# l13039968960/stm32H7-YOLO

Measured on AMD Instinct MI355X. Metric: images/sec int8 YOLO-face 56x56, higher is better.
Workload: dtype int8; 1 GPU; BASELINE configs[1]: batch=4096 int8 YOLO-face 56x56x3 frames per GPU, fused LDS-resident forward + GPU box decode; frames_per_gpu=4096, global_batch=4096, frame_bytes_in=9408, frame_bytes_out=882, input_batches_rotated=8, input_bytes_resident=308281344, kernel=yoloface56_fused<F=2,NW=8>, requant_rounding=ref, parallelism=single GPU, gather_every=1, collectives_issued=0, launch_streams=2

## Files before the change

### stm32h7-yolo_amd/csrc/yf_fused56.hip.h

```cpp


template <class B, int C, int F, int NT>
__device__ __forceinline__ void dump_buf(const char* frames, int8_t* dump, long stride, long off, long first_frame,
                                         long n_frames, int tid, int ch0 = 0, int split = 1 << 30, int gap = 0) {
  if (!dump) return;
  for (int i = tid; i < F * B::P * C; i += NT) {
    const int ch = i % C; const int t = i / C;
    const int p = t % B::P; const int f = t / B::P;
    if (first_frame + f >= n_frames) continue;
    const int phys = ch0 + ch + (ch >= split ? gap : 0);
    dump[(first_frame + f) * stride + off + (long)p * C + ch] = (int8_t)frames[f * B::FS + B::at_p(p) + phys];
  }
}

template <class B, int C, int FT, int NT, class IdOf>
__device__ __forceinline__ void dump_sets(const char* frames, int8_t* dump, long stride, long off, const IdOf& id_of, int tid, int ch0 = 0, int split = 1 << 30, int gap = 0) {
  for (int i = tid; i < FT * B::P * C; i += NT) {
    const int ch = i % C; const int t = i / C;
    const int p = t % B::P; const int f = t / B::P;
    const long id = id_of(f);
    if (id < 0) continue;
    const int phys = ch0 + ch + (ch >= split ? gap : 0);
    dump[id * stride + off + (long)p * C + ch] = (int8_t)frames[f * B::FS + B::at_p(p) + phys];
  }
}

struct DumpOffsets {
  enum { T1 = 0, T2 = T1 + 6272, T3 = T2 + 6272, T4 = T3 + 3136, Q21 = T4 + 14112, T6 = Q21 + 3528, T7 = T6 + 3528,
         T8 = T7 + 1176, T9 = T8 + 7056, T11 = T9 + 7056, T14 = T11 + 1176, T15 = T14 + 7056, Q45 = T15 + 4704,
         T17 = Q45 + 1176, T18 = T17 + 1176, T19 = T18 + 392, T20 = T19 + 1960, T22 = T20 + 1960, T23 = T22 + 392,
         T24 = T23 + 1960, T26 = T24 + 1960, T30 = T26 + 392, T31 = T30 + 2352, T32 = T31 + 1960, T33 = T32 + 1960,
         P8 = T33 + 1568, C17 = P8 + 3528, P25 = C17 + 1176, C34 = P25 + 1176, C40 = C34 + 392, L43 = C40 + 392,
         TOTAL = L43 + 1176 };
};
// ... 44 lines not shown
#endif
template <bool DUMP> constexpr bool tail_batch() { return !DUMP || YF_PDUMP; }

template <int F, int NW, bool DUMP, bool CAM = false>
#if !defined(YF_LAB) || !defined(YF_TPJ13)
#undef YF_TPJ13
#define YF_TPJ13 3
#endif
#if !defined(YF_LAB) || !defined(YF_TPJ23)
#undef YF_TPJ23
#define YF_TPJ23 2
#endif
#if defined(YF_LAB) && defined(YF_WHATIF_WPE)
#define YF_WPE(NW) YF_WHATIF_WPE
#else
#define YF_WPE(NW) ((NW) == 12 ? 6 : (NW) >= 8 ? 4 : ((NW) == 6 ? 3 : 2))
#endif
__global__ void __launch_bounds__(NW * 64, YF_WPE(NW)) yoloface56_fused(const NetParams prm) {
  extern __shared__ __attribute__((aligned(16))) char smem[];
  constexpr int NT = NW * 64;
  constexpr bool BATCH = tail_batch<DUMP>();
  constexpr bool POOL_MERGE = YF_POOL_MERGE != 0 && (!DUMP || YF_PDUMP) && NW >= 8;
  constexpr bool XDUMP = DUMP && !YF_PDUMP;
  typedef Buf<B_T14::OFF, 14, 14, 32, 14, 0, 0> B_T6X;
  typedef typename std::conditional<POOL_MERGE, B_T6X, B_T6>::type B_T6M;
  constexpr int FT = BATCH ? 2 * F : F;
  typedef TailBufs<BATCH ? FRAME_STRIDE / 2 : FRAME_STRIDE> U;
  constexpr int OUT_ALL_BYTES = BATCH ? 0 : (F * OUT_FRAME_BYTES + 15) & ~15;
  static_assert(std::is_same<decltype(&yoloface56_fused<F, NW, DUMP, CAM>), void (*)(const NetParams)>::value, "YF_ARG: NetParams is the kernel's only argument (kernarg offset 0)");
  uint8_t* luts = reinterpret_cast<uint8_t*>(smem);
  constexpr int PRE = v2::pre_bytes<F, tail_batch<DUMP>()>();
  char* out_all = smem + PRE;
  char* frames = smem + PRE + OUT_ALL_BYTES;
  const int n_frames = (int)prm.n;
  const int tid0 = threadIdx.x;
  const uint8_t* __restrict__ tab = prm.tab;
  int vz = 0;
  asm volatile("" : "+v"(vz));
  const __attribute__((address_space(1))) uint8_t* lut_src = (const __attribute__((address_space(1))) uint8_t*)(tab + PLAN.lut_off);
  asm volatile("" : "+s"(lut_src));
  for (int i = tid0; i < v2::LUT_B / 16; i += NT)
    reinterpret_cast<v4u*>(luts)[i] = *(const __attribute__((address_space(1))) v4u*)(lut_src + (uint32_t)(16 * i));
  for (int i = tid0; i < v2::ZERO_B / 16; i += NT) reinterpret_cast<uint4*>(smem + v2::ZERO)[i] = uint4{0, 0, 0, 0};
  constexpr int DBG_LUT = PRE + OUT_ALL_BYTES + FRAME_BYTES + (F - 1) * FRAME_STRIDE;
  if constexpr (DUMP) { if (tid0 < YF_DBG_LUT_BYTES / 16) reinterpret_cast<v4u*>(smem + DBG_LUT)[tid0] = *(const __attribute__((address_space(1))) v4u*)(lut_src + (uint32_t)(YF_N_LUT * 256 + YF_ADDLUT_BYTES + 16 * tid0)); }
#if !(defined(YF_LAB) && defined(YF_WHATIF_NO_PROLOGUE_TABLES))
  {
// ... 385 lines not shown
```

### stm32h7-yolo_amd/csrc/yf_kernels.hip.h

```cpp
#include <hip/hip_runtime.h>
#include <stddef.h>
#include <stdint.h>
#include <type_traits>
#include "yf_tables.h"

#pragma clang diagnostic push
#pragma clang diagnostic ignored "-Wint-to-pointer-cast"
#if !defined(YF_LAB) || !defined(YF_LAUNDER)
#undef YF_LAUNDER
#define YF_LAUNDER 0
#endif
#define YF_ROW_SKEW 4
#define YF_T8_ROW_SKEW 32
namespace YF_NS {

#ifndef YF_NOINLINE_STAGES
#define YF_STAGE_FN __device__ __forceinline__
#else
#define YF_STAGE_FN __device__ __attribute__((noinline))
#endif

typedef int v4i __attribute__((ext_vector_type(4)));
typedef short v2s __attribute__((ext_vector_type(2)));

#if !defined(YF_H0) || YF_H0 == 56
constexpr int FRAME_BYTES = 34176;
#endif
constexpr int LUT_BYTES = YF_N_LUT * 256 + YF_ADDLUT_BYTES;


#if !defined(YF_H0) || YF_H0 == 56
#if defined(YF_LAB) && defined(YF_WHATIF_FS)
constexpr int FRAME_STRIDE = YF_WHATIF_FS;
#else
constexpr int FRAME_STRIDE = FRAME_BYTES;
#endif
constexpr int BUF_FS = FRAME_STRIDE;
#else
constexpr int BUF_FS = 0;
#endif
template <int OFF_, int W_, int H_, int S_, int RS_, int PT_, int PL_, int FS_ = BUF_FS, int SK_ = 0>
struct Buf {
  static constexpr int OFF = OFF_, W = W_, H = H_, S = S_, RS = RS_, PT = PT_, PL = PL_, FS = FS_, SK = SK_;
  static constexpr int P = W_ * H_, ROWB = RS_ * S_ + SK_;
  __device__ static __forceinline__ int at(int y, int x) { return OFF_ + (y + PT_) * ROWB + (x + PL_) * S_; }
  __device__ static __forceinline__ int at_p(int p) {
    if constexpr (RS_ == W_ && PT_ == 0 && PL_ == 0) return OFF_ + p * S_;
    else { const int y = p / W_; return at(y, p - y * W_); }
  }
};
template <int WIDTH>
constexpr bool lds_conflict_free(const int (&addr)[32]) {
  for (int i = 0; i < 32; ++i) {
    if (addr[i] % WIDTH != 0) return false;
    for (int j = 0; j < i; ++j)
      if (addr[i] != addr[j] && (addr[i] / WIDTH) % 32 == (addr[j] / WIDTH) % 32) return false;
  }
  return true;
}

#ifndef YF_H0
#define YF_H0 56
#endif
constexpr int G0 = YF_H0, G1 = G0 / 2, G2 = G0 / 4, G3 = G0 / 8;
static_assert(G0 % 8 == 0 && G3 >= 4, "input size must be a multiple of 8 and at least 32");

#if YF_H0 == 56
typedef Buf<    0, 56, 56,  4, 60, 1, 4> B_IN;
typedef Buf<13696, 28, 28,  8, 30, 1, 1, BUF_FS, YF_ROW_SKEW> B_T1;
typedef Buf<21024, 28, 28,  8, 28, 0, 0> B_T2;
typedef Buf<16832, 28, 28,  4, 28, 0, 0> B_T3;
typedef Buf<    0, 28, 28, 20, 29, 1, 1> B_T4;
typedef Buf<16832, 14, 28, 20, 14, 0, 0> B_HB;
typedef Buf<24672, 14, 14, 48, 14, 0, 0> B_T14;
typedef Buf<16832, 14, 14, 32, 14, 0, 0> B_T6;
typedef Buf<    0, 14, 14,  8, 14, 0, 0> B_T7;
typedef Buf< 1568, 14, 14, 36, 16, 1, 1, BUF_FS, YF_T8_ROW_SKEW> B_T8;
typedef Buf<11296, 14, 14, 48, 14, 0, 0> B_T9;
typedef Buf<20704, 14, 14,  8, 14, 0, 0> B_T11;
typedef Buf<    0, 14, 14, 24, 15, 1, 1> B_T15;
typedef Buf< 5408,  7,  7, 48,  7, 0, 0> B_T30;
typedef Buf< 7760,  7,  7, 32,  7, 0, 0> B_T17;
typedef Buf< 9328,  7,  7,  8,  7, 0, 0> B_T18;
typedef Buf< 9728,  7,  7, 40,  9, 1, 1, BUF_FS, YF_ROW_SKEW> B_T19;
typedef Buf<13008,  7,  7, 48,  7, 0, 0> B_T20;
typedef Buf<15360,  7,  7,  8,  7, 0, 0> B_T22;
typedef Buf<15752,  7,  7,  8,  7, 0, 0> B_T26;
typedef Buf<16144,  7,  7, 32,  7, 0, 0> B_T33;
template <int FS_>
struct TailBufs {
  typedef Buf<    0, 14, 14, 24, 15, 1, 1, FS_> T15;
  typedef Buf< 5408,  7,  7, 48,  7, 0, 0, FS_> T30;
  typedef Buf< 7760,  7,  7, 32,  7, 0, 0, FS_> T17;
  typedef Buf< 9328,  7,  7,  8,  7, 0, 0, FS_> T18;
  typedef Buf< 9728,  7,  7, 40,  9, 1, 1, FS_, YF_ROW_SKEW> T19;
  typedef Buf<13008,  7,  7, 48,  7, 0, 0, FS_> T20;
  typedef Buf<15360,  7,  7,  8,  7, 0, 0, FS_> T22;
  typedef Buf<15752,  7,  7,  8,  7, 0, 0, FS_> T26;
  typedef Buf< 7760,  7,  7, 32,  7, 0, 0, FS_> T33;
  typedef Buf<16160,  7,  7, 18,  7, 0, 0, FS_> HEAD;
  static constexpr int END = 16160 + 882, T15_BYTES = 5408;
  static_assert(T19::OFF + 9 * T19::ROWB <= T20::OFF && T20::OFF + 49 * 48 <= T22::OFF && T26::OFF + 49 * 8 <= HEAD::OFF, "tail buffers do not overlap");
#if !(defined(YF_LAB) && defined(YF_WHATIF_FS))
  static_assert(END <= FS_, "a set fits its stride");
#endif
};
#else
constexpr int arena_next(int off, int bytes) { return (off + bytes + 64 + 63) & ~63; }
#define YF_SEQ(NAME, PREV_END, W_, H_, S_, RS_, PT_, PL_, ROWS_)                      \
  constexpr int NAME##_OFF = PREV_END;                                                \
  typedef Buf<NAME##_OFF, W_, H_, S_, RS_, PT_, PL_> NAME;                            \
  constexpr int NAME##_END = arena_next(NAME##_OFF, (ROWS_) * (RS_) * (S_));
YF_SEQ(B_IN,  0,         G0, G0,  4, G0 + 4, 1, 4, G0 + 1)
YF_SEQ(B_T1,  B_IN_END,  G1, G1,  8, G1 + 2, 1, 1, G1 + 2)
// ... 246 lines not shown
template <int JOBS, int NW>
__device__ __forceinline__ void job_range(int wave, int& j0, int& j1) {
  constexpr int BASE = JOBS / NW, REM = JOBS % NW;
  j0 = wave * BASE + min(wave, REM);
  j1 = j0 + BASE + (wave < REM ? 1 : 0);
}

template <class B, bool RING, int F, int NT>
YF_STAGE_FN void fill_halo(char* frames, int zp, int tid) {
  const uint32_t v = (uint32_t)(zp & 255) * 0x01010101u;
  constexpr int DW = B::S / 4;
  constexpr int HR = B::H + B::PT + (RING ? 1 : 0), WR = B::RS;
  constexpr int NPIX = RING ? (2 * WR + 2 * (HR - 2)) : (WR + HR - 1);
  for (int i = tid; i < F * NPIX * DW; i += NT) {
    const int d = i % DW, t = i / DW, k = t % NPIX, f = t / NPIX;
    int r, c;
    if constexpr (RING) {
      if (k < WR) { r = 0; c = k; }
      else if (k < 2 * WR) { r = HR - 1; c = k - WR; }
      else { const int m = k - 2 * WR; r = 1 + (m >> 1); c = (m & 1) ? WR - 1 : 0; }
    } else {
      if (k < WR) { r = 0; c = k; } else { r = 1 + (k - WR); c = 0; }
    }
    *reinterpret_cast<uint32_t*>(frames + f * B::FS + B::OFF + r * B::ROWB + c * B::S + 4 * d) = v;
  }
}

__device__ __forceinline__ uint32_t funnel(uint32_t hi, uint32_t lo, int sh) { return __builtin_amdgcn_alignbit(hi, lo, sh); }
template <int F, int NT>
YF_STAGE_FN void stage_input(char* frames, const int8_t* __restrict__ in, int first_frame, int n_frames,
                                            int zp, int tid) {
  const uint32_t hv = (uint32_t)(zp & 255) * 0x01010101u;
  constexpr int RSW = B_IN::RS, HH = B_IN::H, WQ = B_IN::W / 4;
  constexpr int PER_FRAME = HH * WQ, TOTAL = F * PER_FRAME, ITERS = (TOTAL + NT - 1) / NT;
  for (int i = tid; i < F * (RSW + HH); i += NT) {
    const int f = i / (RSW + HH), k = i - f * (RSW + HH);
    const int idx = k < RSW ? k : (k - RSW + 1) * RSW + 3;
    *reinterpret_cast<uint32_t*>(frames + f * B_IN::FS + B_IN::OFF + idx * 4) = hv;
  }
  const int lastf = min(n_frames - 1 - first_frame, F - 1);
  const int8_t* base = in + (size_t)(uint32_t)first_frame * IN_FRAME_BYTES;
  static_assert(RSW == B_IN::W + 4 && B_IN::S == 4, "dst = OFF + 16 * (r + y + RSW/4 + 1) relies on rows of W + 4 dwords");
  uint32_t ld[ITERS][3];
#pragma unroll
  for (int it = 0; it < ITERS; ++it) {
    const int i = min(tid + it * NT, TOTAL - 1);
    int f = 0;
// ... 84 lines not shown
template <int NO, int LIM, class LOADC, class STORE>
__device__ __forceinline__ void pool8_sweep(int o0, LOADC loadc, STORE store) {
  constexpr int NR = NO + 3;
  SplitB r[NR];
#pragma unroll
  for (int jj = 0; jj < NR; ++jj) {
    const int j = o0 - 2 + jj;
    r[jj] = SplitB(loadc(clampi(2 * j + 1, 0, LIM))).mx(SplitB(loadc(clampi(2 * j + 2, 0, LIM))));
  }
  SplitB q[NR - 1];
#pragma unroll
  for (int jj = 0; jj < NR - 1; ++jj) q[jj] = r[jj].mx(r[jj + 1]);
#pragma unroll
  for (int n = 0; n < NO; ++n) store(o0 + n, q[n].mx(q[n + 2]));
}
template <int F, int NT>
YF_STAGE_FN void pool8_h(char* frames, int tid) {
  constexpr int NO = 5, OW = B_HB::W, IH = B_T4::H, NCH = (OW + NO - 1) / NO;
  __builtin_assume(tid >= 0 && tid < NT);
  for (int i = tid; i < F * IH * NCH * 5; i += NT) {
    const int cg = i % 5; int t = i / 5;
    const int k = t % NCH; t /= NCH;
    const int y = t % IH; const int f = t / IH;
    char* fbase = frames + f * B_T4::FS;
    const char* row = fbase + B_T4::at(y, 0) + 4 * cg;
    char* dst = fbase + B_HB::OFF + (y * OW) * 20 + 4 * cg;
    pool8_sweep<NO, B_T4::W - 1>(min(k * NO, OW - NO),
                                 [&](int x) { return lds_u32(row + x * B_T4::S); },
                                 [&](int ox, const SplitB& v) { *reinterpret_cast<uint32_t*>(dst + ox * 20) = v.merge(); });
  }
}
#if YF_H0 == 56
template <int F>
constexpr bool pool8_rows_conflict_free(int arena0) {
  constexpr int NO = 5, OW = B_HB::W, IH = B_T4::H;
  if (F != 2 || IH > 32) return false;
  for (int f = 0; f < F; ++f)
    for (int k = 0; k < (OW + NO - 1) / NO; ++k)
      for (int cg = 0; cg < 5; ++cg)
        for (int jj = 0; jj < 2 * (NO + 3); ++jj) {
          const int o0 = k * NO < OW - NO ? k * NO : OW - NO, x0 = 2 * (o0 - 2 + jj / 2) + 1 + jj % 2, x = x0 < 0 ? 0 : x0 > B_T4::W - 1 ? B_T4::W - 1 : x0;
          int addr[32] = {};
          for (int l = 0; l < 32; ++l) {
            const int y = l < IH ? l : IH - 1;
            addr[l] = arena0 + f * B_T4::FS + B_T4::OFF + (y + B_T4::PT) * B_T4::ROWB + (x + B_T4::PL) * B_T4::S + 4 * cg;
          }
          if (!lds_conflict_free<4>(addr)) return false;
        }
  return true;
}
template <int F, int PH>
YF_STAGE_FN void pool8_h_rows(char* frames, int wave, int lane) {
  constexpr int NO = 5, OW = B_HB::W, IH = B_T4::H;
  static_assert(F == 2 && PH == 3 && PH * NO >= OW && IH <= 32, "one wave per chunk of five outputs, one frame per half-wave");
  asm volatile("" : "+v"(lane));
  const int y = lane & 31;
  if (y < IH) {
    char* fbase = frames + (lane >> 5) * B_T4::FS;
    const char* row = fbase + B_T4::at(y, 0);
    char* dst = fbase + B_HB::OFF + y * (OW * 20);
    auto pass = [&](auto o0) {
#pragma nounroll
      for (int cg = 0; cg < 5; ++cg)
        pool8_sweep<NO, B_T4::W - 1>(decltype(o0)::value,
                                     [&](int x) { return lds_u32(row + 4 * cg + x * B_T4::S); },
                                     [&](int ox, const SplitB& v) { *reinterpret_cast<uint32_t*>(dst + 4 * cg + ox * 20) = v.merge(); });
    };
    if (wave == 0) pass(std::integral_constant<int, 0>());
    else if (wave == 1) pass(std::integral_constant<int, NO>());
    else pass(std::integral_constant<int, OW - NO>());
  }
}
#endif
template <int F, int NT, bool STASH = false>
YF_STAGE_FN void pool8_v(char* frames, int tid) {
  constexpr int NO = 5, OW = B_HB::W, OH = B_T14::H, NCH = (OH + NO - 1) / NO;
  static_assert(OH >= NO, "column shorter than one sweep");
  __builtin_assume(tid >= 0 && tid < NT);
  for (int i = tid; i < F * OW * NCH * 5; i += NT) {
    const int cg = i % 5; int t = i / 5;
    const int k = t % NCH; t /= NCH;
    const int ox = t % OW; const int f = t / OW;
    char* fbase = frames + f * B_HB::FS;
// ... 158 lines not shown
  }
  int j0, j1;
  job_range<JOBS, NW>(wave, j0, j1);
  auto run_chunk = [&](const int chunk, int mt, const int n) __attribute__((always_inline)) {
    v4i a[TPJ][KS];
    PassV pv[TPJ];
    PassS ksr[TPJ];
    const uint32_t a_addr = a_lane + (uint32_t)chunk * a_step;
#pragma unroll
    for (int t = 0; t < TPJ; ++t) {
      const int ps = chunk * TPJ + t;
#pragma unroll
      for (int ks = 0; ks < KS; ++ks) a[t][ks] = lds_v4i(a_addr + (uint32_t)(t * 4 * KROW + 16 * ks));
      pv[t].m2 = lds_v4u((uint32_t)(PV + ps * 32));
      pv[t].zr = lds_v4u((uint32_t)(PV + ps * 32 + 16));
      const uint8_t* s = sc + min(ps, NP - 1) * (int)sizeof(yf_pass_s);
      ksr[t] = PassS{*(cv4ul_ptr)(uintptr_t)s, *(cv4i_ptr)(uintptr_t)(s + 32)};
    }
    const int cq = chunk * TPJ * 4;
    const int out_cc = out_c + cq, add_cc = add_c + cq;
    for (int k = 0; k < n; ++k, ++mt) {
      const char* src; char* dstpix = nullptr; const char* addpix = nullptr; char* headpix = nullptr; char* stashpix = nullptr;
      if constexpr (FRAME_TILES) {
        char* fbase = frames + mt * IN::FS;
        src = fbase + in_c;
        dstpix = fbase + out_cc; addpix = fbase + add_cc;
        if constexpr (STASH_OFF >= 0) stashpix = fbase + stash_c + cq;
        if constexpr (EPI == EPI_HEAD) headpix = out_all + mt * OUT_FRAME_BYTES + out_c;
        if constexpr (EPI == EPI_HEAD_LDS) headpix = fbase + OUT::OFF + out_c;
      } else {
        const int q = min(mt * 64 + lane, TOT - 1);
        int f = 0;
#pragma unroll
        for (int i = 1; i < F; ++i) f += (q >= i * P) ? 1 : 0;
        const int p = q - f * P;
        char* fbase = frames + f * IN::FS;
        src = fbase + IN::OFF + p * IN::S;
        if constexpr (EPI == EPI_HEAD) headpix = out_all + f * OUT_FRAME_BYTES + p * 18;
        else if constexpr (EPI == EPI_HEAD_LDS) headpix = fbase + OUT::OFF + p * 18;
        else if constexpr (OUT::RS == OUT::W && OUT::PT == 0 && OUT::PL == 0) dstpix = fbase + cq + OUT::OFF + p * OUT::S + OUT_CH0;
        else { const int y = DivW<OUT::W>::div(p); dstpix = fbase + cq + OUT::at(y, p - y * OUT::W) + OUT_CH0; }
        if constexpr (EPI == EPI_ADD) addpix = fbase + cq + ADDB::OFF + p * ADDB::S;
        if constexpr (STASH_OFF >= 0) stashpix = fbase + cq + STASH_OFF + p * STASH_S;
      }
      v4i b[KS];
#pragma unroll
      for (int ks = 0; ks < KS - 1; ++ks) b[ks] = *reinterpret_cast<const v4i*>(src + 16 * ks);
      const char* last = src + 16 * (KS - 1);
      if constexpr (BW == 16) b[KS - 1] = *reinterpret_cast<const v4i*>(last);
      else if constexpr (BW == 8) { const int2 t2 = *reinterpret_cast<const int2*>(last); b[KS - 1] = v4i{t2.x, t2.y, any_value(), any_value()}; }
      else b[KS - 1] = v4i{*reinterpret_cast<const int*>(last), any_value(), any_value(), any_value()};
#pragma unroll
      for (int t = 0; t < TPJ; ++t) {
        const int ps = chunk * TPJ + t;
        if (ps < NP) {
          v4i acc = acc_init(pv[t].zr);
#pragma unroll
          for (int ks = 0; ks < KS; ++ks) acc = __builtin_amdgcn_mfma_i32_16x16x64_i8(a[t][ks], b[ks], acc, 0, 0, 0);
          constexpr bool HALF_L = YF_HALF_PASS && COUT % 4 == 2 && STASH_OFF < 0 && (EPI == EPI_LUT || EPI == EPI_RAW || EPI == EPI_ADD);
          const bool half = HALF_L && t == (NP - 1) % TPJ && ps == NP - 1;
          if (half) {
            if constexpr (HALF_L) {
              int idx2[2];
              requant2<true, DENSE_SIGNLESS, RQ_FP32>(acc, pv[t].m2, pv[t].zr, ksr[t].c64, ksr[t].rs, idx2);
              epilogue2_half<EPI, LUT_ID, LA>(dstpix, addpix, t * 4, idx2, ad);
            }
// ... 9 lines not shown
  if constexpr (NCH <= YF_CHUNK_UNROLL) {
#pragma unroll
    for (int chunk = 0; chunk < NCH; ++chunk) {
      const int lo = max(j0, chunk * MT), hi = min(j1, (chunk + 1) * MT);
      if (lo < hi) run_chunk(chunk, lo - chunk * MT, hi - lo);
    }
  } else {
    int chunk = (int)((uint32_t)j0 / (uint32_t)MT), mt = j0 - chunk * MT, left = j1 - j0;
    while (left > 0) {
      const int n = min(left, MT - mt);
      run_chunk(chunk, mt, n);
      left -= n; ++chunk; mt = 0;
    }
  }
}

template <int F, class IN, class OUT>
constexpr bool conv1_pairs_conflict_free(int arena0) {
  if (IN::RS % 2 != 0) return false;
  for (int q0 = 0; q0 < F * OUT::P; q0 += 32) {
    int addr[32] = {};
    for (int l = 0; l < 32; ++l) {
      const int q = q0 + l < F * OUT::P ? q0 + l : F * OUT::P - 1, f = q / OUT::P, p = q - f * OUT::P, oy = p / OUT::W, ox = p - oy * OUT::W;
      addr[l] = arena0 + f * IN::FS + IN::OFF + 4 * (2 * oy * IN::RS + 2 * ox + 4);
    }
    if (!lds_conflict_free<8>(addr)) return false;
  }
  return true;
}
template <int F, int NW, int CS, class IN = B_IN, class OUT = B_T1, class LAY = Lay56>
YF_STAGE_FN void conv1_2_stage(char* frames, const uint8_t* __restrict__ tab, int wave, int lane) {
  constexpr int P = OUT::P, W1 = OUT::W, RSW = IN::RS, TOT = F * P;
  constexpr int MT = (TOT + 63) / 64;
  constexpr int SLOT = LAY::slot(CS), WB = plan_wbytes(CS), PV = SLOT + WB;
  const int g = lane >> 4, c = lane & 15;
  const bool a_on = (c >> 2) == g;
  const uint32_t a_addr = a_on ? (uint32_t)(SLOT + (c & 3) * YF_CONV1_KROW) : (uint32_t)LAY::ZERO;
  const uint8_t* sc = tab + PLAN.sb_off[CS];
  static_assert(RSW % 2 == 0 && IN::OFF % 8 == 0 && IN::FS % 8 == 0, "the tap pairs (kx = 1, 2) of a kernel row are 8-byte aligned");
  v4i a[2][3];
  PassV pv[2];
#pragma unroll
  for (int ps = 0; ps < 2; ++ps) {
    v4i t[3];
#pragma unroll
    for (int ks = 0; ks < 3; ++ks) t[ks] = lds_v4i(a_addr + (uint32_t)(ps * 4 * YF_CONV1_KROW + 16 * ks));
    a[ps][0] = v4i{t[0][0], t[0][3], t[0][1], t[0][2]};
// ... 14 lines not shown
    const int oy = DivW<W1>::div(p), ox = p - oy * W1;
    char* fbase = frames + f * IN::FS;
    const uint32_t* src = reinterpret_cast<const uint32_t*>(fbase + IN::OFF) + (2 * oy * RSW + 2 * ox + 3);
    const uint2 r0 = *reinterpret_cast<const uint2*>(src + 1), r1 = *reinterpret_cast<const uint2*>(src + RSW + 1), r2 = *reinterpret_cast<const uint2*>(src + 2 * RSW + 1);
    const v4i b0 = {(int)src[0], (int)src[RSW], (int)r0.x, (int)r0.y};
    const v4i b1 = {(int)r1.x, (int)r1.y, (int)r2.x, (int)r2.y};
    const v4i b2 = {(int)src[2 * RSW], any_value(), any_value(), any_value()};
    char* dstpix = fbase + OUT::at(oy, ox);
#pragma unroll
    for (int ps = 0; ps < 2; ++ps) {
      const uint8_t* s = sc + ps * (int)sizeof(yf_pass_s);
      const PassS k = PassS{*(cv4ul_ptr)(uintptr_t)s, *(cv4i_ptr)(uintptr_t)(s + 32)};
      v4i acc = acc_init(pv[ps].zr);
      acc = __builtin_amdgcn_mfma_i32_16x16x64_i8(a[ps][0], b0, acc, 0, 0, 0);
      acc = __builtin_amdgcn_mfma_i32_16x16x64_i8(a[ps][1], b1, acc, 0, 0, 0);
      acc = __builtin_amdgcn_mfma_i32_16x16x64_i8(a[ps][2], b2, acc, 0, 0, 0);
      int idx[4];
      requant4<true, DENSE_SIGNLESS, RQ_FP32>(acc, pv[ps].m2, pv[ps].zr, k.c64, k.rs, idx);
      epilogue2<EPI_LUT, YF_L_LEAKY2, 0>(dstpix, nullptr, nullptr, 4 * ps, 0, idx, ad);
    }
  }
}

struct DwWalk { int R, FG; };
template <int F, int STRIDE, int W, int H>
constexpr DwWalk dw_rows_per_lane() {
#if YF_H0 == 56
  if (STRIDE == 1 && F == 2 && W == 28 && H == 28) return DwWalk{7, 1};
  if (STRIDE == 1 && F == 2 && W == 14 && H == 14) return DwWalk{2, 1};
  if (STRIDE == 2 && F == 2 && W == 14 && H == 14) return DwWalk{7, 2};
  if (STRIDE == 2 && F == 4 && W == 7 && H == 7) return DwWalk{4, 2};
#endif
  return DwWalk{1, 1};
}
template <int F, int STRIDE, class IN, class OUT>
struct DwGeo {
  static constexpr int W = OUT::W, H = OUT::H;
  static constexpr DwWalk WK = dw_rows_per_lane<F, STRIDE, OUT::W, OUT::H>();
  static constexpr int R = WK.R, FG = WK.FG, RG = 4 / FG, BR = RG * R;
  static constexpr int FL = (W <= 8 && F % 2 == 0) ? 2 : 1;
  static constexpr int NSEG = (W + 15) / 16, NRB = (H + BR - 1) / BR, NFP = F / (FL * FG);
  static constexpr int JPG = NFP * NRB * NSEG;
  static_assert(OUT::RS == W && OUT::PT == 0 && OUT::PL == 0, "depthwise outputs are plain buffers");
  static_assert(IN::FS == OUT::FS, "one frame stride per stage");
  static_assert((H >= BR || (R > 1 && H >= R)) && (W >= 16 || W * FL <= 16) && F % (FL * FG) == 0 && RG * FG == 4, "tile shape");
  static constexpr int seg_row_c(int rs) { return BR > H && rs * R > H - R ? H - R : rs * R; }
  __device__ static __forceinline__ int seg_row(int rs) { return BR > H ? min(rs * R, H - R) : rs * R; }
  static constexpr bool taps_conflict_free() {
    for (int half = 0; half < 2; ++half) {
      int addr[32] = {};
      for (int l = 0; l < 32; ++l) {
        const int g = 2 * half + l / 16, c = l % 16;
        const int fl = FL == 2 ? c / 8 : 0, xc = FL == 2 ? c % 8 : c, xl = xc < W - 1 ? xc : W - 1;
        addr[l] = (fl + FL * (g / RG)) * IN::FS + seg_row_c(g % RG) * STRIDE * IN::ROWB + xl * STRIDE * IN::S;
      }
      if (!lds_conflict_free<4>(addr)) return false;
    }
    return true;
  }
  __device__ static __forceinline__ uint2 job(int jj) {
    const int fp = jj / (NRB * NSEG); int rem = jj - fp * (NRB * NSEG);
    const int rb = rem / NSEG, seg = rem - rb * NSEG;
    const int oy0 = BR > H ? 0 : min(rb * BR, H - BR);
    const int x0 = (W >= 16) ? min(seg * 16, W - 16) : 0;
    const int fb = fp * FL * FG * IN::FS;
    return uint2{(uint32_t)(fb + IN::OFF + (oy0 * STRIDE) * IN::ROWB + x0 * STRIDE * IN::S), (uint32_t)(fb + OUT::OFF + (oy0 * W + x0) * OUT::S)};
  }
};
#if YF_H0 == 56
template <int F, bool BATCH>
struct JobTabs {
  typedef TailBufs<BATCH ? FRAME_STRIDE / 2 : FRAME_STRIDE> U;
  static constexpr int FT = BATCH ? 2 * F : F;
  static constexpr int JT_DW3 = 0;
  static constexpr int JT_DW10 = JT_DW3 + 8 * DwGeo<F, 1, B_T1, B_T2>::JPG;
  static constexpr int JT_DW15 = JT_DW10 + 8 * DwGeo<F, 2, B_T4, B_T6>::JPG;
  static constexpr int JT_DW27 = JT_DW15 + 8 * DwGeo<F, 1, B_T8, B_T9>::JPG;
  static constexpr int JT_DW32 = JT_DW27 + 8 * DwGeo<FT, 2, typename U::T15, typename U::T17>::JPG;
  static constexpr int END = JT_DW32 + 8 * DwGeo<FT, 1, typename U::T19, typename U::T20>::JPG;
  static_assert(END <= JT_B, "job tables fit");
};
#endif
template <class B, bool RING, int F>
struct HaloGeo {
  static constexpr int HR = B::H + B::PT + (RING ? 1 : 0), WR = B::RS;
  static constexpr int NPIX = RING ? (2 * WR + 2 * (HR - 2)) : (WR + HR - 1);
  static constexpr int N = F * NPIX;
  static_assert(B::S % 4 == 0 && B::OFF % 4 == 0 && B::FS % 4 == 0, "dword pixels");
  __device__ static __forceinline__ uint32_t entry(int i) {
    const int f = i / NPIX, k = i - f * NPIX;
    int r, c;
    if constexpr (RING) {
      if (k < WR) { r = 0; c = k; }
      else if (k < 2 * WR) { r = HR - 1; c = k - WR; }
      else { const int m = k - 2 * WR; r = 1 + (m >> 1); c = (m & 1) ? WR - 1 : 0; }
    } else {
      if (k < WR) { r = 0; c = k; } else { r = 1 + (k - WR); c = 0; }
    }
    return (uint32_t)(f * B::FS + B::OFF + r * B::ROWB + c * B::S);
  }
};
#if YF_H0 == 56
template <int F, bool BATCH>
struct HaloTabs {
  typedef TailBufs<BATCH ? FRAME_STRIDE / 2 : FRAME_STRIDE> U;
  static constexpr int FT = BATCH ? 2 * F : F;
  typedef HaloGeo<B_T1, true, F> G1; typedef HaloGeo<B_T4, false, F> G4; typedef HaloGeo<B_T8, true, F> G8;
  typedef HaloGeo<B_T15, false, F> G15; typedef HaloGeo<typename U::T19, true, FT> G19;
  static constexpr int H_T1 = 0, H_T4 = H_T1 + 2 * G1::N, H_T8 = H_T4 + 2 * G4::N, H_T15 = H_T8 + 2 * G8::N, H_T19 = H_T15 + 2 * G15::N;
  static constexpr int BYTES = (H_T19 + 2 * G19::N + 15) & ~15;
};
constexpr int HT = SLOT0 + 2 * SLOT_B;
template <int F, bool BATCH> constexpr int pre_bytes() { return HT + HaloTabs<F, BATCH>::BYTES; }
#if !(defined(YF_LAB) && defined(YF_WHATIF_FS))
static_assert(DwGeo<2, 1, B_T1, B_T2>::taps_conflict_free(), "conv2d_3: the tap reads of a half-wave fall on distinct LDS banks");
static_assert(DwGeo<2, 1, B_T8, B_T9>::taps_conflict_free(), "conv2d_15: the tap reads of a half-wave fall on distinct LDS banks");
static_assert(conv1_pairs_conflict_free<2, B_IN, B_T1>(pre_bytes<2, true>()) && conv1_pairs_conflict_free<2, B_IN, B_T1>(pre_bytes<2, false>()) &&
              conv1_pairs_conflict_free<1, B_IN, B_T1>(pre_bytes<1, true>()) && conv1_pairs_conflict_free<1, B_IN, B_T1>(pre_bytes<1, false>()),
              "conv2d_1: the tap pairs of a half-wave fall on distinct LDS bank pairs");
static_assert(pool8_rows_conflict_free<2>(pre_bytes<2, true>()) && pool8_rows_conflict_free<2>(pre_bytes<2, false>()),
              "pool_8 h (rows across the lanes): every read of the sweep puts the rows of a half-wave on distinct LDS banks");
#endif
static_assert(B_T7::OFF + B_T7::P * B_T7::S <= B_T8::OFF && B_T8::OFF + (B_T8::H + 2) * B_T8::ROWB <= B_T9::OFF && B_T9::OFF + B_T9::P * B_T9::S <= B_T11::OFF &&
              B_T11::OFF + B_T11::P * B_T11::S <= B_T14::OFF, "T7 | T8 | T9 | T11 | concat_22 do not overlap");
template <class G, int HOFF, int NT>
__device__ __forceinline__ void build_halotab(char* smem, int tid) {
  for (int i = tid; i < G::N; i += NT) *reinterpret_cast<uint16_t*>(smem + HT + HOFF + 2 * i) = (uint16_t)(G::entry(i) >> 2);
}
template <class B, class G, int HOFF>
YF_STAGE_FN void fill_halo_t(char* frames, int zp, int tid) {
  typedef const __attribute__((address_space(3))) uint16_t* lds_u16_ptr;
  if (tid < G::N) {
    const uint32_t v = (uint32_t)(zp & 255) * 0x01010101u;
    char* p = frames + 4u * (uint32_t)*(lds_u16_ptr)(uint32_t)(HT + HOFF + 2 * tid);
    if constexpr (B::S % 8 == 0 && B::OFF % 8 == 0 && B::FS % 8 == 0) {
#pragma unroll
      for (int d = 0; d < B::S / 8; ++d) *reinterpret_cast<uint2*>(p + 8 * d) = uint2{v, v};
    } else {
#pragma unroll
      for (int d = 0; d < B::S / 4; ++d) *reinterpret_cast<uint32_t*>(p + 4 * d) = v;
    }
  }
}
#endif

template <int F, int STRIDE, class IN, class OUT, int JTOFF, class LAY = Lay56>
__device__ __forceinline__ void fill_jobtab(char* smem, int tid) {
  typedef DwGeo<F, STRIDE, IN, OUT> G;
  static_assert(JTOFF % 8 == 0 && JTOFF + G::JPG * 8 <= LAY::JT_BYTES, "job table in bounds");
  if (tid < G::JPG) *reinterpret_cast<uint2*>(smem + LAY::JT + JTOFF + 8 * tid) = G::job(tid);
}

template <int F, int NW, int STRIDE, class IN, class OUT, int C, int LUT_ID, int CS, int JTOFF, class LAY = Lay56>
YF_STAGE_FN void dw2_stage(char* frames, const uint8_t* __restrict__ tab, int wave, int lane) {
  typedef DwGeo<F, STRIDE, IN, OUT> G;
  constexpr int W = G::W, FL = G::FL, JPG = G::JPG;
  constexpr int NG = (C + 3) / 4, JOBS = NG * JPG;
  constexpr int DROW = STRIDE * IN::ROWB;
  constexpr int TS = IN::S, TR = IN::ROWB;
  constexpr int SLOT = LAY::slot(CS);
  static_assert(yf_cs_dw[CS] >= 0 && NG == plan_passes(CS), "stage and constant block agree");
  const int g = lane >> 4, c = lane & 15;
  const int fl = (FL == 2) ? (c >> 3) : 0;
  const int xl = (FL == 2) ? min(c & 7, W - 1) : min(c, W - 1);
  const int fr = fl + FL * (g / G::RG), row0 = G::seg_row(g % G::RG);
  const char* lane_in = frames + fr * IN::FS + row0 * DROW + xl * STRIDE * IN::S;
  char* lane_out = frames + fr * IN::FS + (row0 * W + xl) * OUT::S;
  const bool a_on = (c >> 2) == g;
  const uint32_t a_lane = a_on ? (uint32_t)(SLOT + 4 * (c & 3)) : (uint32_t)LAY::ZERO;
  const uint32_t a_step = a_on ? (uint32_t)YF_DWV_GROUP_BYTES : 0u;
  const uint8_t* sc = tab + PLAN.sb_off[CS];
  int j, j1;
  job_range<JOBS, NW>(wave, j, j1);
  int cg = (int)((uint32_t)j / (uint32_t)JPG), jj = j - cg * JPG, left = j1 - j;
  while (left > 0) {
    const uint32_t wa = a_lane + (uint32_t)cg * a_step;
    v4i a0, a1, a2 = {0, 0, 0, 0};
    a0 = v4i{(int)*(lds_u32_ptr)(wa), (int)*(lds_u32_ptr)(wa + 16), (int)*(lds_u32_ptr)(wa + 32), (int)*(lds_u32_ptr)(wa + 48)};
    a1 = v4i{(int)*(lds_u32_ptr)(wa + 64), (int)*(lds_u32_ptr)(wa + 80), (int)*(lds_u32_ptr)(wa + 96), (int)*(lds_u32_ptr)(wa + 112)};
    a2[0] = (int)*(lds_u32_ptr)(wa + 128);
    PassV pv;
    pv.m2 = lds_v4u((uint32_t)(SLOT + cg * YF_DWV_GROUP_BYTES + 144));
    pv.zr = lds_v4u((uint32_t)(SLOT + cg * YF_DWV_GROUP_BYTES + 160));
    const uint8_t* s = sc + cg * (int)sizeof(yf_pass_s);
    const PassS k = PassS{*(cv4ul_ptr)(uintptr_t)s, *(cv4i_ptr)(uintptr_t)(s + 32)};
    const char* lin = lane_in + 4 * cg;
    char* lout = lane_out + 4 * cg;
    auto entry = [&](int job) { return *(lds_u2_ptr)(uint32_t)(LAY::JT + JTOFF + 8 * min(job, JPG - 1)); };
    auto taps = [&](const v2u e, v4i& b0, v4i& b1, v4i& b2, char*& dst) {
      const char* src = lin + e[0];
// ... 56 lines not shown
      taps(e1, q0, q1, q2, dq);
      e0 = entry(jj + i + 2); e1 = entry(jj + i + 3);
      const v4i ap = conv(p0, p1, p2);
      const v4i aq = conv(q0, q1, q2);
      finish(ap, dp);
      finish(aq, dq);
    }
    if (i < n) {
      v4i b0, b1, b2 = {0, any_value(), any_value(), any_value()};
      char* dst;
      taps(e0, b0, b1, b2, dst);
      finish(conv(b0, b1, b2), dst);
    }
    left -= n; ++cg; jj = 0;
  }
}
template <int FT> constexpr int pool25_waves() { return (FT * 42 + 63) / 64; }
template <int FT, class T15, class T30, bool STASH = false>
YF_STAGE_FN void pool25_cols(char* frames, int item) {
  static_assert(T15::W == 14 && T15::H == 14 && T30::W == 7 && T15::FS == T30::FS, "pool_25 geometry");
  const int t = DivW<6>::div(item), cg = item - 6 * t;
  const int f = DivW<7>::div(t), ox = t - 7 * f;
  if (f >= FT) return;
  char* fbase = frames + f * T15::FS;
  const char* base = fbase + T15::at(0, 0) + 4 * cg;
  constexpr int S = T15::S, ROW = T15::ROWB;
  const int c0 = max(2 * ox - 1, 0) * S, c1 = 2 * ox * S, c2 = c1 + S, c3 = min(2 * ox + 2, 13) * S;
  auto hrow = [&](int r) {
    const char* p = base + r * ROW;
    return SplitB(lds_u32(p + c0)).mx(SplitB(lds_u32(p + c1))).mx(SplitB(lds_u32(p + c2))).mx(SplitB(lds_u32(p + c3)));
  };
  char* dst = fbase + T30::OFF + ox * T30::S + 4 * cg;
  SplitB prev = hrow(0);
#pragma unroll
  for (int oy = 0; oy < 7; ++oy) {
    SplitB next = hrow(2 * oy + 1);
    if (2 * oy + 2 <= 13) next = next.mx(hrow(2 * oy + 2));
    const SplitB mxv = prev.mx(next);
    *reinterpret_cast<uint32_t*>(dst + oy * (7 * T30::S)) = lut4_raw<YF_L_Q45>(mxv);
    if constexpr (STASH) *reinterpret_cast<uint32_t*>(dst + oy * (7 * T30::S) + 24) = mxv.merge();
    prev = next;
  }
}
}
#ifndef YF_GENERIC
#include "yf_fused56.hip.h"
#else
#ifdef YF_LAB
// ... 8 lines not shown
```

Baseline: 33.13 million images/s.

## Add per-frame LDS skews to T4, T15, T6X buffers to cut bank conflicts

Adds a per-frame byte skew (FK) to several LDS activation buffers so that the second frame of a pair lands on different banks. All addressing paths (halo zeroing, depthwise tap walks, pooling, pointwise epilogues, dumps) go through a new frame_off helper. It also reorders the depthwise lane-group mapping for stride-2 stages so that groups interleave frames. Static asserts check that the stride-2 depthwise taps are conflict-free or at most 2-way. The intent is to remove LDS bank conflicts in conv2d_10, conv2d_27 and the pool stages, at the cost of more address arithmetic and a risk of layout overlap bugs.

```diff
diff --git a/stm32h7-yolo_amd/csrc/yf_fused56.hip.h b/stm32h7-yolo_amd/csrc/yf_fused56.hip.h
--- a/stm32h7-yolo_amd/csrc/yf_fused56.hip.h
+++ b/stm32h7-yolo_amd/csrc/yf_fused56.hip.h
@@ -9,7 +9,7 @@
     const int p = t % B::P; const int f = t / B::P;
     if (first_frame + f >= n_frames) continue;
     const int phys = ch0 + ch + (ch >= split ? gap : 0);
-    dump[(first_frame + f) * stride + off + (long)p * C + ch] = (int8_t)frames[f * B::FS + B::at_p(p) + phys];
+    dump[(first_frame + f) * stride + off + (long)p * C + ch] = (int8_t)frames[B::frame_off(f, F) + B::at_p(p) + phys];
   }
 }
 
@@ -100,7 +100,7 @@
   constexpr bool BATCH = tail_batch<DUMP>();
   constexpr bool POOL_MERGE = YF_POOL_MERGE != 0 && (!DUMP || YF_PDUMP) && NW >= 8;
   constexpr bool XDUMP = DUMP && !YF_PDUMP;
-  typedef Buf<B_T14::OFF, 14, 14, 32, 14, 0, 0> B_T6X;
+  static_assert(B_T6X::OFF == B_T14::OFF && B_T6X::OFF + B_T6X::P * B_T6X::S + B_T6X::FK <= B_T14::OFF + B_T14::P * B_T14::S, "conv2d_10's output, skew included, on concat_22's bytes");
   typedef typename std::conditional<POOL_MERGE, B_T6X, B_T6>::type B_T6M;
   constexpr int FT = BATCH ? 2 * F : F;
   typedef TailBufs<BATCH ? FRAME_STRIDE / 2 : FRAME_STRIDE> U;
diff --git a/stm32h7-yolo_amd/csrc/yf_kernels.hip.h b/stm32h7-yolo_amd/csrc/yf_kernels.hip.h
--- a/stm32h7-yolo_amd/csrc/yf_kernels.hip.h
+++ b/stm32h7-yolo_amd/csrc/yf_kernels.hip.h
@@ -11,6 +11,9 @@
 #define YF_LAUNDER 0
 #endif
 #define YF_ROW_SKEW 4
+#define YF_T4_FRAME_SKEW 4
+#define YF_T15_FRAME_SKEW 4
+#define YF_T6X_FRAME_SKEW 16
 #define YF_T8_ROW_SKEW 32
 namespace YF_NS {
 
@@ -39,9 +42,13 @@
 #else
 constexpr int BUF_FS = 0;
 #endif
-template <int OFF_, int W_, int H_, int S_, int RS_, int PT_, int PL_, int FS_ = BUF_FS, int SK_ = 0>
+template <int OFF_, int W_, int H_, int S_, int RS_, int PT_, int PL_, int FS_ = BUF_FS, int SK_ = 0, int FK_ = 0, int FKD_ = 1>
 struct Buf {
-  static constexpr int OFF = OFF_, W = W_, H = H_, S = S_, RS = RS_, PT = PT_, PL = PL_, FS = FS_, SK = SK_;
+  static constexpr int OFF = OFF_, W = W_, H = H_, S = S_, RS = RS_, PT = PT_, PL = PL_, FS = FS_, SK = SK_, FK = FK_, FKD = FKD_, FP = FS_ + FK_;
+  static constexpr bool skewed(int frames) { return FK_ != 0 && frames == 2 * FKD_; }
+  static constexpr int frame_off(int f, int frames) {
+    return !skewed(frames) ? f * FS_ : FKD_ == 1 ? f * (FS_ + FK_) : f * FS_ + (f / FKD_) * FK_;
+  }
   static constexpr int P = W_ * H_, ROWB = RS_ * S_ + SK_;
   __device__ static __forceinline__ int at(int y, int x) { return OFF_ + (y + PT_) * ROWB + (x + PL_) * S_; }
   __device__ static __forceinline__ int at_p(int p) {
@@ -70,15 +77,18 @@
 typedef Buf<13696, 28, 28,  8, 30, 1, 1, BUF_FS, YF_ROW_SKEW> B_T1;
 typedef Buf<21024, 28, 28,  8, 28, 0, 0> B_T2;
 typedef Buf<16832, 28, 28,  4, 28, 0, 0> B_T3;
-typedef Buf<    0, 28, 28, 20, 29, 1, 1> B_T4;
+typedef Buf<    0, 28, 28, 20, 29, 1, 1, BUF_FS, 0, YF_T4_FRAME_SKEW> B_T4;
+static_assert(B_T4::OFF + (B_T4::H + B_T4::PT) * B_T4::ROWB + B_T4::FK <= 16832, "the skewed T4 ends in front of T3 / HB");
 typedef Buf<16832, 14, 28, 20, 14, 0, 0> B_HB;
 typedef Buf<24672, 14, 14, 48, 14, 0, 0> B_T14;
 typedef Buf<16832, 14, 14, 32, 14, 0, 0> B_T6;
+typedef Buf<24672, 14, 14, 32, 14, 0, 0, BUF_FS, 0, YF_T6X_FRAME_SKEW> B_T6X;
 typedef Buf<    0, 14, 14,  8, 14, 0, 0> B_T7;
 typedef Buf< 1568, 14, 14, 36, 16, 1, 1, BUF_FS, YF_T8_ROW_SKEW> B_T8;
 typedef Buf<11296, 14, 14, 48, 14, 0, 0> B_T9;
 typedef Buf<20704, 14, 14,  8, 14, 0, 0> B_T11;
-typedef Buf<    0, 14, 14, 24, 15, 1, 1> B_T15;
+typedef Buf<    0, 14, 14, 24, 15, 1, 1, BUF_FS, 0, YF_T15_FRAME_SKEW> B_T15;
+static_assert(B_T15::OFF + (B_T15::H + B_T15::PT) * B_T15::ROWB + B_T15::FK <= 5408, "the skewed T15 stays inside its 5 408-byte block (the park copies whole blocks) and in front of concat_46");
 typedef Buf< 5408,  7,  7, 48,  7, 0, 0> B_T30;
 typedef Buf< 7760,  7,  7, 32,  7, 0, 0> B_T17;
 typedef Buf< 9328,  7,  7,  8,  7, 0, 0> B_T18;
@@ -89,7 +99,7 @@
 typedef Buf<16144,  7,  7, 32,  7, 0, 0> B_T33;
 template <int FS_>
 struct TailBufs {
-  typedef Buf<    0, 14, 14, 24, 15, 1, 1, FS_> T15;
+  typedef Buf<    0, 14, 14, 24, 15, 1, 1, FS_, 0, YF_T15_FRAME_SKEW, FRAME_STRIDE / FS_> T15;
   typedef Buf< 5408,  7,  7, 48,  7, 0, 0, FS_> T30;
   typedef Buf< 7760,  7,  7, 32,  7, 0, 0, FS_> T17;
   typedef Buf< 9328,  7,  7,  8,  7, 0, 0, FS_> T18;
@@ -382,7 +392,7 @@
     } else {
       if (k < WR) { r = 0; c = k; } else { r = 1 + (k - WR); c = 0; }
     }
-    *reinterpret_cast<uint32_t*>(frames + f * B::FS + B::OFF + r * B::ROWB + c * B::S + 4 * d) = v;
+    *reinterpret_cast<uint32_t*>(frames + B::frame_off(f, F) + B::OFF + r * B::ROWB + c * B::S + 4 * d) = v;
   }
 }
 
@@ -513,8 +523,8 @@
     const int cg = i % 5; int t = i / 5;
     const int k = t % NCH; t /= NCH;
     const int y = t % IH; const int f = t / IH;
-    char* fbase = frames + f * B_T4::FS;
-    const char* row = fbase + B_T4::at(y, 0) + 4 * cg;
+    char* fbase = frames + f * B_HB::FS;
+    const char* row = fbase + (B_T4::skewed(F) ? f * B_T4::FK : 0) + B_T4::at(y, 0) + 4 * cg;
     char* dst = fbase + B_HB::OFF + (y * OW) * 20 + 4 * cg;
     pool8_sweep<NO, B_T4::W - 1>(min(k * NO, OW - NO),
                                  [&](int x) { return lds_u32(row + x * B_T4::S); },
@@ -534,7 +544,7 @@
           int addr[32] = {};
           for (int l = 0; l < 32; ++l) {
             const int y = l < IH ? l : IH - 1;
-            addr[l] = arena0 + f * B_T4::FS + B_T4::OFF + (y + B_T4::PT) * B_T4::ROWB + (x + B_T4::PL) * B_T4::S + 4 * cg;
+            addr[l] = arena0 + f * B_T4::FP + B_T4::OFF + (y + B_T4::PT) * B_T4::ROWB + (x + B_T4::PL) * B_T4::S + 4 * cg;
           }
           if (!lds_conflict_free<4>(addr)) return false;
         }
@@ -547,9 +557,8 @@
   asm volatile("" : "+v"(lane));
   const int y = lane & 31;
   if (y < IH) {
-    char* fbase = frames + (lane >> 5) * B_T4::FS;
-    const char* row = fbase + B_T4::at(y, 0);
-    char* dst = fbase + B_HB::OFF + y * (OW * 20);
+    const char* row = frames + (lane >> 5) * B_T4::FP + B_T4::at(y, 0);
+    char* dst = frames + (lane >> 5) * B_HB::FP + B_HB::OFF + y * (OW * 20);
     auto pass = [&](auto o0) {
 #pragma nounroll
       for (int cg = 0; cg < 5; ++cg)
@@ -754,6 +763,7 @@
     for (int k = 0; k < n; ++k, ++mt) {
       const char* src; char* dstpix = nullptr; const char* addpix = nullptr; char* headpix = nullptr; char* stashpix = nullptr;
       if constexpr (FRAME_TILES) {
+        static_assert(IN::FK == 0 && OUT::FK == 0 && ADDB::FK == 0, "no frame skews on the 7x7 grid");
         char* fbase = frames + mt * IN::FS;
         src = fbase + in_c;
         dstpix = fbase + out_cc; addpix = fbase + add_cc;
@@ -766,14 +776,17 @@
 #pragma unroll
         for (int i = 1; i < F; ++i) f += (q >= i * P) ? 1 : 0;
         const int p = q - f * P;
-        char* fbase = frames + f * IN::FS;
+        static_assert(IN::FKD == 1 && OUT::FKD == 1 && ADDB::FKD == 1, "one skew step per frame on the 28x28 and 14x14 grids");
+        constexpr int IFK = IN::skewed(F) ? IN::FK : 0, OFK = OUT::skewed(F) ? OUT::FK : 0, AFK = ADDB::skewed(F) ? ADDB::FK : 0;
+        char* fbase = frames + f * (IN::FS + IFK);
+        char* obase = fbase + f * (OFK - IFK);
         src = fbase + IN::OFF + p * IN::S;
         if constexpr (EPI == EPI_HEAD) headpix = out_all + f * OUT_FRAME_BYTES + p * 18;
-        else if constexpr (EPI == EPI_HEAD_LDS) headpix = fbase + OUT::OFF + p * 18;
-        else if constexpr (OUT::RS == OUT::W && OUT::PT == 0 && OUT::PL == 0) dstpix = fbase + cq + OUT::OFF + p * OUT::S + OUT_CH0;
-        else { const int y = DivW<OUT::W>::div(p); dstpix = fbase + cq + OUT::at(y, p - y * OUT::W) + OUT_CH0; }
-        if constexpr (EPI == EPI_ADD) addpix = fbase + cq + ADDB::OFF + p * ADDB::S;
-        if constexpr (STASH_OFF >= 0) stashpix = fbase + cq + STASH_OFF + p * STASH_S;
+        else if constexpr (EPI == EPI_HEAD_LDS) headpix = obase + OUT::OFF + p * 18;
+        else if constexpr (OUT::RS == OUT::W && OUT::PT == 0 && OUT::PL == 0) dstpix = obase + cq + OUT::OFF + p * OUT::S + OUT_CH0;
+        else { const int y = DivW<OUT::W>::div(p); dstpix = obase + cq + OUT::at(y, p - y * OUT::W) + OUT_CH0; }
+        if constexpr (EPI == EPI_ADD) addpix = fbase + f * (AFK - IFK) + cq + ADDB::OFF + p * ADDB::S;
+        if constexpr (STASH_OFF >= 0) stashpix = fbase - f * IFK + cq + STASH_OFF + p * STASH_S;
       }
       v4i b[KS];
 #pragma unroll
@@ -829,7 +842,7 @@
     int addr[32] = {};
     for (int l = 0; l < 32; ++l) {
       const int q = q0 + l < F * OUT::P ? q0 + l : F * OUT::P - 1, f = q / OUT::P, p = q - f * OUT::P, oy = p / OUT::W, ox = p - oy * OUT::W;
-      addr[l] = arena0 + f * IN::FS + IN::OFF + 4 * (2 * oy * IN::RS + 2 * ox + 4);
+      addr[l] = arena0 + f * IN::FP + IN::OFF + 4 * (2 * oy * IN::RS + 2 * ox + 4);
     }
     if (!lds_conflict_free<8>(addr)) return false;
   }
@@ -890,22 +903,25 @@
   }
 }
 
-struct DwWalk { int R, FG; };
+struct DwWalk { int R, FG; bool FF; };
 template <int F, int STRIDE, int W, int H>
 constexpr DwWalk dw_rows_per_lane() {
 #if YF_H0 == 56
-  if (STRIDE == 1 && F == 2 && W == 28 && H == 28) return DwWalk{7, 1};
-  if (STRIDE == 1 && F == 2 && W == 14 && H == 14) return DwWalk{2, 1};
-  if (STRIDE == 2 && F == 2 && W == 14 && H == 14) return DwWalk{7, 2};
-  if (STRIDE == 2 && F == 4 && W == 7 && H == 7) return DwWalk{4, 2};
-#endif
-  return DwWalk{1, 1};
+  if (STRIDE == 1 && F == 2 && W == 28 && H == 28) return DwWalk{7, 1, false};
+  if (STRIDE == 1 && F == 2 && W == 14 && H == 14) return DwWalk{2, 1, false};
+  if (STRIDE == 2 && F == 2 && W == 14 && H == 14) return DwWalk{7, 2, true};
+  if (STRIDE == 2 && F == 4 && W == 7 && H == 7) return DwWalk{4, 2, true};
+#endif
+  return DwWalk{1, 1, false};
 }
 template <int F, int STRIDE, class IN, class OUT>
 struct DwGeo {
   static constexpr int W = OUT::W, H = OUT::H;
   static constexpr DwWalk WK = dw_rows_per_lane<F, STRIDE, OUT::W, OUT::H>();
   static constexpr int R = WK.R, FG = WK.FG, RG = 4 / FG, BR = RG * R;
+  static constexpr bool FF = WK.FF;
+  static constexpr int grp_frame(int g) { return FF ? g % FG : g / RG; }
+  static constexpr int grp_seg(int g) { return FF ? g / FG : g % RG; }
   static constexpr int FL = (W <= 8 && F % 2 == 0) ? 2 : 1;
   static constexpr int NSEG = (W + 15) / 16, NRB = (H + BR - 1) / BR, NFP = F / (FL * FG);
   static constexpr int JPG = NFP * NRB * NSEG;
@@ -914,25 +930,36 @@
   static_assert((H >= BR || (R > 1 && H >= R)) && (W >= 16 || W * FL <= 16) && F % (FL * FG) == 0 && RG * FG == 4, "tile shape");
   static constexpr int seg_row_c(int rs) { return BR > H && rs * R > H - R ? H - R : rs * R; }
   __device__ static __forceinline__ int seg_row(int rs) { return BR > H ? min(rs * R, H - R) : rs * R; }
-  static constexpr bool taps_conflict_free() {
+  static constexpr bool taps_conflict_free() { return taps_ways() == 1; }
+  static constexpr int taps_ways() {
+    int worst = 0;
     for (int half = 0; half < 2; ++half) {
       int addr[32] = {};
       for (int l = 0; l < 32; ++l) {
         const int g = 2 * half + l / 16, c = l % 16;
         const int fl = FL == 2 ? c / 8 : 0, xc = FL == 2 ? c % 8 : c, xl = xc < W - 1 ? xc : W - 1;
-        addr[l] = (fl + FL * (g / RG)) * IN::FS + seg_row_c(g % RG) * STRIDE * IN::ROWB + xl * STRIDE * IN::S;
+        addr[l] = IN::frame_off(fl + FL * grp_frame(g), F) + seg_row_c(grp_seg(g)) * STRIDE * IN::ROWB + xl * STRIDE * IN::S;
       }
-      if (!lds_conflict_free<4>(addr)) return false;
-    }
-    return true;
+      for (int i = 0; i < 32; ++i) {
+        int k = 0;
+        for (int j = 0; j < 32; ++j) {
+          bool first = (addr[j] / 4) % 32 == (addr[i] / 4) % 32;
+          for (int m = 0; m < j && first; ++m) first = addr[m] != addr[j];
+          k += first ? 1 : 0;
+        }
+        worst = k > worst ? k : worst;
+      }
+    }
+    return worst;
   }
   __device__ static __forceinline__ uint2 job(int jj) {
     const int fp = jj / (NRB * NSEG); int rem = jj - fp * (NRB * NSEG);
     const int rb = rem / NSEG, seg = rem - rb * NSEG;
     const int oy0 = BR > H ? 0 : min(rb * BR, H - BR);
     const int x0 = (W >= 16) ? min(seg * 16, W - 16) : 0;
-    const int fb = fp * FL * FG * IN::FS;
-    return uint2{(uint32_t)(fb + IN::OFF + (oy0 * STRIDE) * IN::ROWB + x0 * STRIDE * IN::S), (uint32_t)(fb + OUT::OFF + (oy0 * W + x0) * OUT::S)};
+    const int f0 = fp * FL * FG;
+    return uint2{(uint32_t)(IN::frame_off(f0, F) + IN::OFF + (oy0 * STRIDE) * IN::ROWB + x0 * STRIDE * IN::S),
+                 (uint32_t)(OUT::frame_off(f0, F) + OUT::OFF + (oy0 * W + x0) * OUT::S)};
   }
 };
 #if YF_H0 == 56
@@ -954,7 +981,8 @@
   static constexpr int HR = B::H + B::PT + (RING ? 1 : 0), WR = B::RS;
   static constexpr int NPIX = RING ? (2 * WR + 2 * (HR - 2)) : (WR + HR - 1);
   static constexpr int N = F * NPIX;
-  static_assert(B::S % 4 == 0 && B::OFF % 4 == 0 && B::FS % 4 == 0, "dword pixels");
+  static constexpr int ALIGN = (B::S % 8 == 0 && B::OFF % 8 == 0 && B::frame_off(1, F) % 8 == 0) ? 8 : 4;
+  static_assert(B::S % 4 == 0 && B::OFF % 4 == 0 && B::frame_off(1, F) % 4 == 0, "dword pixels");
   __device__ static __forceinline__ uint32_t entry(int i) {
     const int f = i / NPIX, k = i - f * NPIX;
     int r, c;
@@ -965,7 +993,7 @@
     } else {
       if (k < WR) { r = 0; c = k; } else { r = 1 + (k - WR); c = 0; }
     }
-    return (uint32_t)(f * B::FS + B::OFF + r * B::ROWB + c * B::S);
+    return (uint32_t)(B::frame_off(f, F) + B::OFF + r * B::ROWB + c * B::S);
   }
 };
 #if YF_H0 == 56
@@ -983,6 +1011,8 @@
 #if !(defined(YF_LAB) && defined(YF_WHATIF_FS))
 static_assert(DwGeo<2, 1, B_T1, B_T2>::taps_conflict_free(), "conv2d_3: the tap reads of a half-wave fall on distinct LDS banks");
 static_assert(DwGeo<2, 1, B_T8, B_T9>::taps_conflict_free(), "conv2d_15: the tap reads of a half-wave fall on distinct LDS banks");
+static_assert(DwGeo<2, 2, B_T4, B_T6X>::taps_conflict_free(), "conv2d_10: the tap reads of a half-wave fall on distinct LDS banks");
+static_assert(DwGeo<4, 2, TailBufs<FRAME_STRIDE / 2>::T15, TailBufs<FRAME_STRIDE / 2>::T17>::taps_ways() == 2, "conv2d_27: the tap reads of a half-wave are 2-way conflicts at most");
 static_assert(conv1_pairs_conflict_free<2, B_IN, B_T1>(pre_bytes<2, true>()) && conv1_pairs_conflict_free<2, B_IN, B_T1>(pre_bytes<2, false>()) &&
               conv1_pairs_conflict_free<1, B_IN, B_T1>(pre_bytes<1, true>()) && conv1_pairs_conflict_free<1, B_IN, B_T1>(pre_bytes<1, false>()),
               "conv2d_1: the tap pairs of a half-wave fall on distinct LDS bank pairs");
@@ -1001,7 +1031,7 @@
   if (tid < G::N) {
     const uint32_t v = (uint32_t)(zp & 255) * 0x01010101u;
     char* p = frames + 4u * (uint32_t)*(lds_u16_ptr)(uint32_t)(HT + HOFF + 2 * tid);
-    if constexpr (B::S % 8 == 0 && B::OFF % 8 == 0 && B::FS % 8 == 0) {
+    if constexpr (G::ALIGN == 8) {
 #pragma unroll
       for (int d = 0; d < B::S / 8; ++d) *reinterpret_cast<uint2*>(p + 8 * d) = uint2{v, v};
     } else {
@@ -1031,9 +1061,9 @@
   const int g = lane >> 4, c = lane & 15;
   const int fl = (FL == 2) ? (c >> 3) : 0;
   const int xl = (FL == 2) ? min(c & 7, W - 1) : min(c, W - 1);
-  const int fr = fl + FL * (g / G::RG), row0 = G::seg_row(g % G::RG);
-  const char* lane_in = frames + fr * IN::FS + row0 * DROW + xl * STRIDE * IN::S;
-  char* lane_out = frames + fr * IN::FS + (row0 * W + xl) * OUT::S;
+  const int fr = fl + FL * G::grp_frame(g), row0 = G::seg_row(G::grp_seg(g));
+  const char* lane_in = frames + IN::frame_off(fr, F) + row0 * DROW + xl * STRIDE * IN::S;
+  char* lane_out = frames + OUT::frame_off(fr, F) + (row0 * W + xl) * OUT::S;
   const bool a_on = (c >> 2) == g;
   const uint32_t a_lane = a_on ? (uint32_t)(SLOT + 4 * (c & 3)) : (uint32_t)LAY::ZERO;
   const uint32_t a_step = a_on ? (uint32_t)YF_DWV_GROUP_BYTES : 0u;
@@ -1136,8 +1166,8 @@
   const int t = DivW<6>::div(item), cg = item - 6 * t;
   const int f = DivW<7>::div(t), ox = t - 7 * f;
   if (f >= FT) return;
-  char* fbase = frames + f * T15::FS;
-  const char* base = fbase + T15::at(0, 0) + 4 * cg;
+  char* fbase = frames + f * T30::FS;
+  const char* base = frames + T15::frame_off(f, FT) + T15::at(0, 0) + 4 * cg;
   constexpr int S = T15::S, ROW = T15::ROWB;
   const int c0 = max(2 * ox - 1, 0) * S, c1 = 2 * ox * S, c2 = c1 + S, c3 = min(2 * ox + 2, 13) * S;
   auto hrow = [&](int r) {
```

Result: no change. 33.30 million images/s (median of 6 runs) (+0.5%).
